# tigert1998/ray-tracing-cuda

Hardware: AMD Instinct MI355X
Metric: Mrays/s (higher is better)
Workload: dtype f32

## Files before the change

ray-tracing-cuda_amd/csrc/closest_hit.h:

```cpp
#pragma once

#ifdef RTMI_CHECK_MARGINS
__device__ inline bool aabb_hit_reference(const BvhNode &nd, V3 o, V3 d, double t_from, double t_to) {
  const float oo[3] = {o.x, o.y, o.z}, dd[3] = {d.x, d.y, d.z};
  for (int i = 0; i < 3; i++) {
    if (dd[i] == 0.f) continue;
    for (int s = 0; s < 2; s++) {
      const float tf = ((s == 0 ? nd.mn[i] : nd.mx[i]) - oo[i]) / dd[i];
      const double t = (double)tf;
      if (t != t || fabs(t) == (double)INFINITY) continue;
      if (!(t_from <= t && t <= t_to)) continue;
      const float pt[3] = {oo[0] + (float)t * dd[0], oo[1] + (float)t * dd[1], oo[2] + (float)t * dd[2]};
      bool inside = true;
      for (int a = 0; a < 3; a++)
        if (a != i && !(nd.mn[a] <= pt[a] && pt[a] <= nd.mx[a])) inside = false;
      if (inside) return true;
    }
  }
  return false;
}
template <typename T>
__device__ inline bool bvh_reference_walk(const SceneDev &sc, const BvhRec &br, V3 o, V3 d, T &t_to, int &face, float &fu,
                                          float &fv) {
  int stk_node[kRefDepthMax + 2], stk_first[kRefDepthMax + 2], stk_n[kRefDepthMax + 2];
  int sp = 1;
  stk_node[0] = br.root, stk_first[0] = 0, stk_n[0] = br.n_faces;
  bool hit = false;
  while (sp > 0) {
    sp--;
    const int node = stk_node[sp], first = stk_first[sp], n = stk_n[sp];
    const BvhNode nd = sc.nodes[node];
    if (node != br.root && !aabb_hit_reference(nd, o, d, 1e-3, (double)t_to)) continue;
    if (nd.right < 0) {
      for (int i = 0; i < n; i++) {
        const int fi = sc.face_of_orig[br.face_base + first + i];
        const FaceRec &f = sc.faces[fi];
        float t = 0.f, u = 0.f, v = 0.f;
        if (tri_test<T>(mk(f.p0[0], f.p0[1], f.p0[2]), mk(f.e1[0], f.e1[1], f.e1[2]), mk(f.e2[0], f.e2[1], f.e2[2]), o, d,
                        t_to, t, u, v))
          t_to = (T)t, face = fi, fu = u, fv = v, hit = true;
      }
    } else if (sp + 2 <= kRefDepthMax + 2) {
      const int mid = (n - 1) / 2;
      stk_node[sp] = nd.right, stk_first[sp] = first + mid + 1, stk_n[sp] = n - mid - 1;
      stk_node[sp + 1] = nd.left, stk_first[sp + 1] = first, stk_n[sp + 1] = mid + 1;
      sp += 2;
    }
  }
  return hit;
}
#endif

template <uint32_t M, bool PAIR = false>
__device__ __forceinline__ bool load_tri_pts(const SceneDev &sc, const float4 *s_tris, int rec, int which, V3 &p0, V3 &e1, V3 &e2) {
  float4 qa, qb, qc;
  bool present;
  if ((M & PIN_LDS_TABLES) || s_tris != nullptr) {
    const float4 *pp = s_tris + (size_t)rec * 3;
    if (trims_mul24(M)) {
      uint32_t at = (uint32_t)(uintptr_t)s_tris + __umul24((uint32_t)(PAIR ? rec - which : rec), 48u);
      asm volatile("" : "+v"(at));
      pp = (const float4 *)(const RT_LDS float4 *)(uintptr_t)at + (PAIR ? 3 * which : 0);
    }
    qa = load_lds<float4>(pp), qb = load_lds<float4>(pp + 1), qc = load_lds<float4>(pp + 2);
    present = !(__float_as_int(qc.y) & TRIPTS_ABSENT);
  } else {
    const float4 *pp = reinterpret_cast<const float4 *>(sc.tris + rec);
    qa = load_global<float4>(pp), qb = load_global<float4>(pp + 1), qc = load_global<float4>(pp + 2);
    const float4 qd = load_global<float4>(pp + 3);
    present = which == 0 || (__float_as_int(qd.y) & TRI_SECOND);
  }
  p0 = mk(qa.x, qa.y, qa.z), e1 = mk(qa.w, qb.x, qb.y), e2 = mk(qb.z, qb.w, qc.x);
  return present;
}

template <uint32_t F, bool OCC = false, uint32_t M = 0>
__device__ __forceinline__ Hit closest_hit(const SceneDev &sc, const BvhNode *s_nodes, int lds_nodes, const int *s_paths,
                                           int lds_paths, const float4 *s_tris, int *ll, uint16_t *cands, int *wl,
                                           unsigned long long *overflow, V3 o, V3 d, bool live, bool count_work
#ifdef RTMI_STATS
                                           , MeshStats &st
#endif
                                           , double t_start = INFINITY, double t_stop = INFINITY, bool *uncertain = nullptr
) {
  constexpr bool DT = (F & F_SPHERE) != 0;
  typedef typename TSel<DT>::type T;
  bool ok = false;
  T t_to = OCC ? (T)t_start : (T)INFINITY;
#define RTMI_DECIDED (OCC && ok && t_to <= (T)t_stop)
  uint32_t win = ID_NONE;
  int32_t aux = 0;
  int32_t work = 0;
  float bu = 0.f, bv = 0.f;

  double sa = 0.0, sa2 = 0.0;
  float saf = 0.f;
  if (F & F_SPHERE) {
    float la = len3(d);
    saf = la * la;
    sa = (double)saf;
    sa2 = 2 * sa;
  }

  const int lane = (int)(threadIdx.x & 63u);
  const bool det_safe = (M & PIN_DET_SAFE) || sc.det_safe != 0;
  constexpr bool SLAB = culls_by_slab(M);
  constexpr bool MINF = folds_by_min(M);
  constexpr bool VOTE = trims_votes(M);
  static_assert(!MINF || (!OCC && !DT && !(F & F_TEX)), "a key holds a binary32 t and the triangle's place, nothing else");
  const bool cull_list = (F & F_TRIS) && ((M & PIN_LDS_TABLES) || (ll != nullptr && sc.n_pairs >= kCullMinPairs));
  V3 cull_inv = splat(0.f), cull_klo = splat(0.f), cull_khi = splat(0.f);
  if ((F & F_TRIS) && cull_list) {
    const float ix = __builtin_amdgcn_rcpf(d.x), iy = __builtin_amdgcn_rcpf(d.y), iz = __builtin_amdgcn_rcpf(d.z);
    cull_inv = mk(fabsf(d.x) < 1e-30f ? copysignf(1e30f, d.x) : ix, fabsf(d.y) < 1e-30f ? copysignf(1e30f, d.y) : iy,
                  fabsf(d.z) < 1e-30f ? copysignf(1e30f, d.z) : iz);
    if (SLAB) {
      cull_klo = mk(-o.x * cull_inv.x, -o.y * cull_inv.y, -o.z * cull_inv.z);
    } else {
      const float delta = MESH_DIST_SLACK * (fmaxf(fmaxf(fabsf(o.x), fabsf(o.y)), fabsf(o.z)) + sc.list_mag);
      cull_klo = mk(-(o.x + delta) * cull_inv.x, -(o.y + delta) * cull_inv.y, -(o.z + delta) * cull_inv.z);
      cull_khi = mk(-(o.x - delta) * cull_inv.x, -(o.y - delta) * cull_inv.y, -(o.z - delta) * cull_inv.z);
    }
  }

  for (int ri = 0; ri < sc.n_runs; ri++) {
    if (OCC) {
      live = live && !RTMI_DECIDED;
      if (__builtin_amdgcn_ballot_w64(live) == 0ull) break;
    }
    const i32x4 rv = load_run(sc.runs, ri);
    Run run;
    run.kind = rv[0], run.first = rv[1], run.count = rv[2], run.pad = rv[3];
    if (live && run.kind == RUN_SKY) {
      const T ts = (T)1e9f;
      bool hit = ts <= t_to;
      bool acc = hit && (!ok || ts < t_to);
      ok = ok || acc;
      t_to = acc ? ts : t_to;
      win = acc ? make_id(RUN_SKY, 0) : win;
    }
    if ((F & F_TRIS) && run.kind == RUN_TRIS && cull_list) {
      const int pair0 = run.first >> 1;
      const float lo0 = T_FROM_F * kTimeLo;
      for (int c0 = 0; c0 < run.count; c0 += 32) {
        if (OCC && __builtin_amdgcn_ballot_w64(live && !RTMI_DECIDED) == 0ull) break;
        const int nc = run.count - c0 < 32 ? run.count - c0 : 32;
        const float hi0 = (float)t_to * kTimeHi + kTimeAbs;
        uint32_t mask = 0u;
        RTMI_STAT2(const unsigned long long tc0 = stat_now();)
#define RTMI_CULL_PAIR(bx)                                                                                                      \
  {                                                                                                                             \
    const float t0x = __builtin_fmaf(bx[0], cull_inv.x, cull_klo.x), t1x = __builtin_fmaf(bx[3], cull_inv.x, cull_khi.x); \
    const float t0y = __builtin_fmaf(bx[1], cull_inv.y, cull_klo.y), t1y = __builtin_fmaf(bx[4], cull_inv.y, cull_khi.y); \
    const float t0z = __builtin_fmaf(bx[2], cull_inv.z, cull_klo.z), t1z = __builtin_fmaf(bx[5], cull_inv.z, cull_khi.z); \
    const float en = fmaxf(fmaxf(fminf(t0x, t1x), fminf(t0y, t1y)), fminf(t0z, t1z));                                            \
    const float le = fminf(fminf(fmaxf(t0x, t1x), fmaxf(t0y, t1y)), fmaxf(t0z, t1z));                                            \
    cull_step(mask, fmaxf(lo0, en), fminf(hi0, le));                                                                            \
  }
#define RTMI_CULL_SLAB(bx)                                                                                                      \
  {                                                                                                                             \
    const float tcx = __builtin_fmaf(bx[0], cull_inv.x, cull_klo.x), tcy = __builtin_fmaf(bx[1], cull_inv.y, cull_klo.y),       \
                tcz = __builtin_fmaf(bx[2], cull_inv.z, cull_klo.z);                                                            \
    const float nx = __builtin_fmaf(-bx[3], fabsf(cull_inv.x), tcx), fx = __builtin_fmaf(bx[3], fabsf(cull_inv.x), tcx);        \
    const float ny = __builtin_fmaf(-bx[4], fabsf(cull_inv.y), tcy), fy = __builtin_fmaf(bx[4], fabsf(cull_inv.y), tcy);        \
    const float nz = __builtin_fmaf(-bx[5], fabsf(cull_inv.z), tcz), fz = __builtin_fmaf(bx[5], fabsf(cull_inv.z), tcz);        \
    const float en = fmaxf(fmaxf(nx, ny), nz), le = fminf(fminf(fx, fy), fz);                                                   \
    cull_step_nlt(mask, fminf(hi0, le), fmaxf(lo0, en));                                                                        \
  }
#define RTMI_CULL_ONE(bx)  \
  if (SLAB) RTMI_CULL_SLAB(bx) else RTMI_CULL_PAIR(bx)
        const PairBox *const recs = sc.pair_boxes;
        f32x8 A = load_pair_box(recs, pair0 + c0), B;
        int i = 0;
        for (; i + 1 < nc; i += 2) {
          __builtin_amdgcn_s_waitcnt(0xc07f);
          __builtin_amdgcn_sched_barrier(0);
          B = load_pair_box(recs, pair0 + c0 + i + 1);
          __builtin_amdgcn_sched_barrier(0);
          RTMI_CULL_ONE(A)
          __builtin_amdgcn_s_waitcnt(0xc07f);
          __builtin_amdgcn_sched_barrier(0);
          A = load_pair_box(recs, pair0 + c0 + i + 2);
          __builtin_amdgcn_sched_barrier(0);
          RTMI_CULL_ONE(B)
        }
        if (i < nc) {
          __builtin_amdgcn_s_waitcnt(0xc07f);
          __builtin_amdgcn_sched_barrier(0);
          RTMI_CULL_ONE(A)
        }
#undef RTMI_CULL_ONE
#undef RTMI_CULL_SLAB
#undef RTMI_CULL_PAIR
        mask = __brev(mask) >> (32 - nc);
        if (!live) mask = 0u;
        if (OCC && RTMI_DECIDED) mask = 0u;
        RTMI_STAT2(const unsigned long long tc1 = stat_now(); st.cyc[5] += tc1 - tc0;)
        RTMI_STAT(st.cull_bits += (unsigned)__popcll(__builtin_amdgcn_ballot_w64(true)) * 0u; { unsigned pc = __builtin_popcount(mask); for (int off = 32; off > 0; off >>= 1) pc += __shfl_down(pc, off); st.cull_bits += __builtin_amdgcn_readfirstlane(pc); } st.cull_rays += (unsigned)__popcll(__builtin_amdgcn_ballot_w64(true));)
#ifndef RTMI_OWN_FIRST
#define RTMI_OWN_FIRST 1
#endif
#if RTMI_OWN_FIRST
        if (wave_ballot_nz<VOTE>(mask) != 0ull) {
          if (mask != 0u) {
            const int bit = __builtin_ctz(mask);
            mask &= mask - 1u;
            const int rec = 2 * (pair0 + c0 + bit);
            V3 p0, e1, e2, p1, e1b, e2b;
            (void)load_tri_pts<M, true>(sc, s_tris, rec, 0, p0, e1, e2);
            const bool second = load_tri_pts<M, true>(sc, s_tris, rec + 1, 1, p1, e1b, e2b);
            float ta = 0.f, ua = 0.f, va = 0.f, tb = 0.f, ub = 0.f, vb = 0.f;
            const bool hit_a = tri_test_flat<T, VOTE>(p0, e1, e2, cross3(d, e2), o, d, t_to, ta, ua, va, det_safe);
            bool hit_b = false;
            if (second) hit_b = tri_test_flat<T, VOTE>(p1, e1b, e2b, cross3(d, e2b), o, d, t_to, tb, ub, vb, det_safe) && !hit_a;
            const float t = hit_a ? ta : tb;
            const bool acc = (hit_a || hit_b) && (!ok || (T)t < t_to);
            ok = ok || acc;
            t_to = acc ? (T)t : t_to;
            win = acc ? make_id(RUN_TRIS, run.first + 2 * (c0 + bit) + (hit_a ? 0 : 1)) : win;
            if (F & F_TEX) {
              bu = acc ? (hit_a ? ua : ub) : bu;
              bv = acc ? (hit_a ? va : vb) : bv;
            }
          }
        }
        if (OCC && RTMI_DECIDED) mask = 0u;
#endif
        {
          constexpr int RW = (F & F_TEX) ? 6 : 2;
          int *tasks = ll + 64 * 8, *results = ll + 64 * 8 + kListTasks(F);
          const int cnt = __builtin_popcount(mask);
          const int base = wave_prefix_excl(cnt);
          if (cnt != 0) {
            int *rr = ll + lane * 8;
            int w3 = 0, w7 = 0;
            if (DT) {
              const double td = (double)t_to;
              w3 = __double2loint(td), w7 = __double2hiint(td);
            } else {
              w3 = __float_as_int((float)t_to);
            }
            *reinterpret_cast<int4 *>(rr) = make_int4(__float_as_int(o.x), __float_as_int(o.y), __float_as_int(o.z), w3);
            *reinterpret_cast<int4 *>(rr + 4) = make_int4(__float_as_int(d.x), __float_as_int(d.y), __float_as_int(d.z), w7);
          }
          bool todo = cnt != 0;
          uint32_t left = (uint32_t)cnt;
#define RTMI_TODO_LANES (VOTE ? wave_ballot_nz<true>(left) : __builtin_amdgcn_ballot_w64(todo))
          while (RTMI_TODO_LANES != 0ull) {
            RTMI_STAT(st.cull_iters++;)
            const int lo_t = __builtin_amdgcn_readlane(base, __builtin_ctzll(RTMI_TODO_LANES));
            const bool now = (VOTE ? left != 0u : todo) && base + cnt - lo_t <= kListTasks(F);
            const unsigned long long now_lanes = VOTE ? RTMI_TODO_LANES & __builtin_amdgcn_sicmp(base + cnt - lo_t, kListTasks(F), 41)
                                                      : __builtin_amdgcn_ballot_w64(now);
            const int n_now = __builtin_amdgcn_readlane(base + cnt, 63 - __builtin_clzll(now_lanes)) - lo_t;
            RTMI_STAT(st.nnow_hist[(n_now - 1) >> 5 < 5 ? (n_now - 1) >> 5 : 5]++;)
            RTMI_STAT({
              int pc = now ? cnt : 0;
              for (int off = 32; off > 0; off >>= 1) pc = max(pc, __shfl_xor(pc, off));
              st.trip_hist[pc < 8 ? pc - 1 : 7]++;
            })
            int ln = lane;
            if (MINF) asm volatile("" : "+v"(ln));
            if (now) {
              int k = base - lo_t;
              for (uint32_t m = mask; m != 0u; m &= m - 1u) tasks[k++] = (lane << 5) | __builtin_ctz(m);
              if (MINF) results[2 * ln + 1] = -1;
            }
            wave_lds_fence();
            if (MINF) {
              bool flagged = false;
              for (int t0 = 0; t0 < 2 * n_now; t0 += 64) {
                const int ti = t0 + ln;
                if (ti < 2 * n_now) {
                  const int w = tasks[ti >> 1], which = ti & 1;
                  const int *orr = ll + (w >> 5) * 8;
                  const float4 r0 = *reinterpret_cast<const float4 *>(orr), r1 = *reinterpret_cast<const float4 *>(orr + 4);
                  const V3 ro = mk(r0.x, r0.y, r0.z), rd = mk(r1.x, r1.y, r1.z);
                  V3 p0, e1, e2;
                  const bool present = load_tri_pts<M>(sc, s_tris, 2 * (pair0 + c0 + (w & 31)) + which, which, p0, e1, e2);
                  float tt = 0.f, uu, vv;
                  bool hit = false;
                  if (present) hit = tri_test_flat<T, VOTE>(p0, e1, e2, cross3(rd, e2), ro, rd, (T)r0.w, tt, uu, vv, det_safe);
                  const int mine = hit ? __float_as_int(tt) : -1;
                  const int other = __builtin_amdgcn_update_dpp(mine, mine, 0xb1, 0xf, 0xf, false);
                  const bool yield = other != -1 && (which != 0 || __int_as_float(other) < tt);
                  flagged = flagged || (hit && yield && which == 0);
                  if (hit && !yield) {
                    const unsigned long long key = ((unsigned long long)(uint32_t)mine << 32) | (uint32_t)(2 * (w & 31) + which);
                    (void)__hip_atomic_fetch_min(reinterpret_cast<unsigned long long *>(results + 2 * (w >> 5)), key,
                                                 __ATOMIC_RELAXED, __HIP_MEMORY_SCOPE_WAVEFRONT);
                  }
                }
              }
              wave_lds_fence();
              const unsigned long long fl = __builtin_amdgcn_ballot_w64(flagged);
              if (fl == 0ull) {
                if (now) {
                  const int2 key = *reinterpret_cast<const int2 *>(results + 2 * ln);
                  const float t = __int_as_float(key.y);
                  const bool acc = key.y != -1 && (!ok || (T)t < t_to);
                  ok = ok || acc;
                  t_to = acc ? (T)t : t_to;
                  win = acc ? make_id(RUN_TRIS, run.first + 2 * c0 + key.x) : win;
                  todo = false, left = 0u;
                }
                wave_lds_fence();
                continue;
              }
              if (lane == 0) atomicAdd(overflow + (kOrderedTasksWord - 2), (unsigned long long)__popcll(fl));
            }
            for (int t0 = 0; t0 < 2 * n_now; t0 += 64) {
              const int ti = t0 + lane;
              if (ti < 2 * n_now) {
                const int w = tasks[ti >> 1], which = ti & 1;
                const int *orr = ll + (w >> 5) * 8;
                const float4 r0 = *reinterpret_cast<const float4 *>(orr), r1 = *reinterpret_cast<const float4 *>(orr + 4);
                T t0_to;
                if (DT) {
                  t0_to = (T)__hiloint2double(__float_as_int(r1.w), __float_as_int(r0.w));
                } else {
                  t0_to = (T)r0.w;
                }
                const V3 ro = mk(r0.x, r0.y, r0.z), rd = mk(r1.x, r1.y, r1.z);
                V3 p0, e1, e2;
                const bool present = load_tri_pts<M>(sc, s_tris, 2 * (pair0 + c0 + (w & 31)) + which, which, p0, e1, e2);
                float tt = 0.f, uu = 0.f, vv = 0.f;
                bool hit = false;
                if (present) hit = tri_test_flat<T, VOTE>(p0, e1, e2, cross3(rd, e2), ro, rd, t0_to, tt, uu, vv, det_safe);
                int *res = results + (ti >> 1) * RW;
                res[which] = hit ? __float_as_int(tt) : (int)0xffffffff;
                if (F & F_TEX) res[2 + 2 * which] = __float_as_int(uu), res[3 + 2 * which] = __float_as_int(vv);
              }
            }
            wave_lds_fence();
            RTMI_STAT2(const unsigned long long tc2 = stat_now();)
            if (now) {
              int k = base - lo_t;
              for (uint32_t m = mask; m != 0u; m &= m - 1u, k++) {
                const int tri = run.first + 2 * (c0 + __builtin_ctz(m));
                const int *res = results + k * RW;
                const int ia = res[0], ib = res[1];
                const float ta = __int_as_float(ia), tb = __int_as_float(ib);
                const bool hit_a = ia != (int)0xffffffff && (T)ta <= t_to;
                const bool hit_b = !hit_a && ib != (int)0xffffffff && (T)tb <= t_to;
                const float t = hit_a ? ta : tb;
                const bool acc = (hit_a || hit_b) && (!ok || (T)t < t_to);
                ok = ok || acc;
                t_to = acc ? (T)t : t_to;
                win = acc ? make_id(RUN_TRIS, tri + (hit_a ? 0 : 1)) : win;
                if (F & F_TEX) {
                  bu = acc ? __int_as_float(hit_a ? res[2] : res[4]) : bu;
                  bv = acc ? __int_as_float(hit_a ? res[3] : res[5]) : bv;
                }
              }
              todo = false, left = 0u;
            }
            wave_lds_fence();
            RTMI_STAT2(st.cyc[7] += stat_now() - tc2;)
          }
#undef RTMI_TODO_LANES
        }
        RTMI_STAT2(st.cyc[6] += stat_now() - tc1;)
      }
    } else if ((F & F_TRIS) && live && run.kind == RUN_TRIS) {
      const HotTri *base = sc.tris + run.first;
      f32x16 A = load_hot_tri(base, 0);
      for (int i = 0; i < run.count; i++) {
        if (OCC && __builtin_amdgcn_ballot_w64(!RTMI_DECIDED) == 0ull) break;
        __builtin_amdgcn_s_waitcnt(0xc07f);
        __builtin_amdgcn_sched_barrier(0);
        const f32x16 B = load_hot_tri(base, 2 * i + 1);
        __builtin_amdgcn_sched_barrier(0);
        float t = 0.f, u = 0.f, v = 0.f;
        const V3 pv_a = cross3(d, mk(A[6], A[7], A[8]));
        const bool hit_a = tri_test_flat<T>(mk(A[0], A[1], A[2]), mk(A[3], A[4], A[5]), mk(A[6], A[7], A[8]), pv_a, o, d,
                                            t_to, t, u, v, det_safe);
        {
          bool acc = hit_a && (!ok || (T)t < t_to);
          ok = ok || acc;
          t_to = acc ? (T)t : t_to;
          win = acc ? make_id(RUN_TRIS, run.first + 2 * i) : win;
          if (F & F_TEX) {
            bu = acc ? u : bu;
            bv = acc ? v : bv;
          }
        }
        __builtin_amdgcn_s_waitcnt(0xc07f);
        __builtin_amdgcn_sched_barrier(0);
        A = load_hot_tri(base, 2 * i + 2);
        __builtin_amdgcn_sched_barrier(0);
        if (__float_as_int(B[13]) & TRI_SECOND) {
          V3 pv_b = pv_a;
          if (!(__float_as_int(B[13]) & TRI_SAME_E2)) pv_b = cross3(d, mk(B[6], B[7], B[8]));
          bool hit_b = tri_test_flat<T>(mk(B[0], B[1], B[2]), mk(B[3], B[4], B[5]), mk(B[6], B[7], B[8]), pv_b, o, d,
                                        t_to, t, u, v, det_safe);
          hit_b = hit_b && !hit_a;
          bool acc = hit_b && (!ok || (T)t < t_to);
          ok = ok || acc;
          t_to = acc ? (T)t : t_to;
          win = acc ? make_id(RUN_TRIS, run.first + 2 * i + 1) : win;
          if (F & F_TEX) {
            bu = acc ? u : bu;
            bv = acc ? v : bv;
          }
        }
      }
    }
    bool grouped_done = false;
    if ((F & F_SGROUP) && run.kind == RUN_SPHERE && run.pad >= 0 && cands != nullptr) {
      const int n_groups = (run.count + kSphGroupSize - 1) / kSphGroupSize;
      uint16_t *my_cands = cands + lane * kSphCand;
      int *tasks = ll + 64 * 8, *results = ll + 64 * 8 + kListTasks(F);
      int ccnt = 0;
      bool have = false;
      double best_v = 0.0;
      int best_idx = 0;
      {
        int *rr = ll + lane * 8;
        *reinterpret_cast<int4 *>(rr) = make_int4(__float_as_int(o.x), __float_as_int(o.y), __float_as_int(o.z), __float_as_int(saf));
        *reinterpret_cast<int4 *>(rr + 4) = make_int4(__float_as_int(d.x), __float_as_int(d.y), __float_as_int(d.z), 0);
      }
      const float sdelta = kSphDistSlack * fmaxf(fmaxf(fabsf(o.x), fabsf(o.y)), fabsf(o.z));
      const float six = __builtin_amdgcn_rcpf(d.x), siy = __builtin_amdgcn_rcpf(d.y), siz = __builtin_amdgcn_rcpf(d.z);
      const V3 s_inv = mk(fabsf(d.x) < 1e-30f ? copysignf(1e30f, d.x) : six, fabsf(d.y) < 1e-30f ? copysignf(1e30f, d.y) : siy,
                          fabsf(d.z) < 1e-30f ? copysignf(1e30f, d.z) : siz);
      const V3 s_klo = mk(-(o.x + sdelta) * s_inv.x, -(o.y + sdelta) * s_inv.y, -(o.z + sdelta) * s_inv.z);
      const V3 s_khi = mk(-(o.x - sdelta) * s_inv.x, -(o.y - sdelta) * s_inv.y, -(o.z - sdelta) * s_inv.z);
      const float s_lo0 = T_FROM_F * kTimeLo, s_hi0 = (float)t_to * kTimeHi + kTimeAbs;
      const int member0 = __float_as_int(load_sph_group(sc.sph_groups, run.pad)[6]);
      auto flush = [&]() {
        const int cnt = ccnt;
        const int base = wave_prefix_excl(cnt);
        bool todo = cnt != 0;
        while (__builtin_amdgcn_ballot_w64(todo) != 0ull) {
          const int lo_t = __builtin_amdgcn_readlane(base, __builtin_ctzll(__builtin_amdgcn_ballot_w64(todo)));
          const bool now = todo && base + cnt - lo_t <= kListTasks(F);
          const int n_now = __builtin_amdgcn_readlane(base + cnt, 63 - __builtin_clzll(__builtin_amdgcn_ballot_w64(now))) - lo_t;
          if (now)
            for (int j = 0; j < cnt; j++) tasks[base - lo_t + j] = (lane << 16) | (int)my_cands[j];
          wave_lds_fence();
          for (int t0 = 0; t0 < n_now; t0 += 64) {
            const int ti = t0 + lane;
            if (ti < n_now) {
              const int w = tasks[ti];
              const int *orr = ll + (w >> 16) * 8;
              const float4 r0 = *reinterpret_cast<const float4 *>(orr), r1 = *reinterpret_cast<const float4 *>(orr + 4);
              const SphMember *mp = sc.sph_members + member0 + (w & 0xffff);
              const float4 m0 = *reinterpret_cast<const float4 *>(mp);
              const int4 m1 = *reinterpret_cast<const int4 *>(reinterpret_cast<const char *>(mp) + 16);
              const double r2 = __hiloint2double(m1.w, m1.z);
              const V3 ro = mk(r0.x, r0.y, r0.z), rd = mk(r1.x, r1.y, r1.z);
              const double tsa = (double)r0.w, tsa2 = 2 * tsa;
              const V3 oc = ro - mk(m0.x, m0.y, m0.z);
              const double b = (double)(2.0f * dot3(rd, oc));
              const float lc = len3(oc);
              const double c = (double)(lc * lc) - r2;
              const double disc = b * b - 4 * tsa * c;
              double v = __hiloint2double(0x7ff80000, 0);
              if (!(disc < 0)) {
                const double sq = sqrt(disc);
                const double t1 = (-b - sq) / tsa2;
                if (1e-3 <= t1) {
                  v = t1;
                } else {
                  const double t2 = (-b + sq) / tsa2;
                  if (1e-3 <= t2) v = t2;
                }
              }
              int *res = results + ti * 3;
              res[0] = __double2loint(v), res[1] = __double2hiint(v), res[2] = m1.x;
            }
          }
          wave_lds_fence();
          if (now) {
            for (int j = 0; j < cnt; j++) {
              const int *res = results + (base - lo_t + j) * 3;
              const double v = __hiloint2double(res[1], res[0]);
              const int idx = res[2];
              if (v == v && (!have || v < best_v || (v == best_v && idx < best_idx))) have = true, best_v = v, best_idx = idx;
            }
            todo = false;
          }
          wave_lds_fence();
        }
        ccnt = 0;
      };
      int *counts = reinterpret_cast<int *>(cands + 64 * kSphCand);
      counts[lane] = 0;
      bool over = false;
      for (int g0 = 0; g0 < n_groups; g0 += 32) {
        const int ngc = n_groups - g0 < 32 ? n_groups - g0 : 32;
        uint32_t gmask = 0u;
        f32x8 G = load_sph_group(sc.sph_groups, run.pad + g0);
        for (int g = 0; g < ngc; g++) {
          __builtin_amdgcn_s_waitcnt(0xc07f);
          __builtin_amdgcn_sched_barrier(0);
          const f32x8 gb = G;
          G = load_sph_group(sc.sph_groups, run.pad + g0 + g + 1);
          __builtin_amdgcn_sched_barrier(0);
          const float t0x = __builtin_fmaf(gb[0], s_inv.x, s_klo.x), t1x = __builtin_fmaf(gb[3], s_inv.x, s_khi.x);
          const float t0y = __builtin_fmaf(gb[1], s_inv.y, s_klo.y), t1y = __builtin_fmaf(gb[4], s_inv.y, s_khi.y);
          const float t0z = __builtin_fmaf(gb[2], s_inv.z, s_klo.z), t1z = __builtin_fmaf(gb[5], s_inv.z, s_khi.z);
          const float en = fmaxf(fmaxf(fminf(t0x, t1x), fminf(t0y, t1y)), fminf(t0z, t1z));
          const float le = fminf(fminf(fmaxf(t0x, t1x), fmaxf(t0y, t1y)), fmaxf(t0z, t1z));
          cull_step(gmask, fmaxf(s_lo0, en), fminf(s_hi0, le));
        }
        gmask = live ? __brev(gmask) >> (32 - ngc) : 0u;
        const int cnt = __builtin_popcount(gmask);
        const int base = wave_prefix_excl(cnt);
        bool todo = cnt != 0;
        while (__builtin_amdgcn_ballot_w64(todo) != 0ull) {
          const int lo_t = __builtin_amdgcn_readlane(base, __builtin_ctzll(__builtin_amdgcn_ballot_w64(todo)));
          const bool now = todo && base + cnt - lo_t <= kListTasks(F);
          const int n_now = __builtin_amdgcn_readlane(base + cnt, 63 - __builtin_clzll(__builtin_amdgcn_ballot_w64(now))) - lo_t;
          if (now) {
            int k = base - lo_t;
            for (uint32_t m = gmask; m != 0u; m &= m - 1u) tasks[k++] = (lane << 16) | (g0 + __builtin_ctz(m));
          }
          wave_lds_fence();
          for (int t0 = 0; t0 < n_now; t0 += 64) {
            const int ti = t0 + lane;
            if (ti < n_now) {
              const int w = tasks[ti];
              const int owner = w >> 16;
              const int *orr = ll + owner * 8;
              const float4 r0 = *reinterpret_cast<const float4 *>(orr), r1 = *reinterpret_cast<const float4 *>(orr + 4);
              const V3 ro = mk(r0.x, r0.y, r0.z), rd = mk(r1.x, r1.y, r1.z);
              const float ta4 = 4.0f * r0.w;
              const int2 gr = *reinterpret_cast<const int2 *>(reinterpret_cast<const char *>(sc.sph_groups + run.pad + (w & 0xffff)) + 24);
              const int rel = gr.x - member0;
              const float4 *mp = reinterpret_cast<const float4 *>(sc.sph_members + gr.x);
#pragma unroll 4
              for (int i = 0; i < kSphGroupSize; i++) {
                if (i < gr.y) {
                  const float4 mb = mp[2 * i];
                  const V3 oc = ro - mk(mb.x, mb.y, mb.z);
                  const float bf = 2.0f * dot3(rd, oc);
                  const float oc2 = dot3(oc, oc);
                  const float bb = bf * bf;
                  const float disc_f = bb - ta4 * (oc2 - mb.w);
                  const float mag = bb + ta4 * (oc2 + mb.w);
                  if (!(disc_f < -kSphDiscRel * mag)) {
                    const int slot = atomicAdd(&counts[owner], 1);
                    if (slot < kSphCand) {
                      cands[owner * kSphCand + slot] = (uint16_t)(rel + i);
                    } else {
                      over = true;
                    }
                  }
                }
              }
            }
          }
          wave_lds_fence();
          if (now) todo = false;
        }
      }
      const bool overflowed = __any(over);
      if (!overflowed) {
        ccnt = counts[lane];
        flush();
        if (have) {
          const bool hit = best_v <= (double)t_to;
          const bool acc = hit && (!ok || best_v < (double)t_to);
          ok = ok || acc;
          t_to = acc ? (T)best_v : t_to;
          win = acc ? make_id(RUN_SPHERE, best_idx) : win;
        }
        grouped_done = true;
      }
    }
    if ((F & F_SPHERE) && live && run.kind == RUN_SPHERE && !grouped_done) {
      f32x8 nxt = load_sphere(sc.spheres, run.first);
      for (int i = 0; i < run.count; i++) {
        if (OCC && __builtin_amdgcn_ballot_w64(!RTMI_DECIDED) == 0ull) break;
        __builtin_amdgcn_s_waitcnt(0xc07f);
        __builtin_amdgcn_sched_barrier(0);
        const f32x8 cur = nxt;
        nxt = load_sphere(sc.spheres, run.first + i + 1);
        __builtin_amdgcn_sched_barrier(0);
        const double r2 = __hiloint2double(__float_as_int(cur[7]), __float_as_int(cur[6]));
        V3 oc = o - mk(cur[0], cur[1], cur[2]);
        const float bf = 2.0f * dot3(d, oc);
        {
          const float oc2 = dot3(oc, oc), r2f = (float)r2;
          const float disc_f = bf * bf - 4.0f * saf * (oc2 - r2f);
          const float mag = bf * bf + 4.0f * saf * (oc2 + r2f);
          if (!__any(!(disc_f < -kSphDiscRel * mag) && !RTMI_DECIDED)) continue;
        }
        double b = (double)bf;
        float lc = len3(oc);
        double c = (double)(lc * lc) - r2;
        double disc = b * b - 4 * sa * c;
        bool hit = false;
        double t = 0.0;
        if (!(disc < 0)) {
          double sq = sqrt(disc);
          t = (-b - sq) / sa2;
          hit = (1e-3 <= t && t <= (double)t_to);
          if (!hit) {
            t = (-b + sq) / sa2;
            hit = (1e-3 <= t && t <= (double)t_to);
          }
        }
        bool acc = hit && (!ok || t < (double)t_to);
        ok = ok || acc;
        t_to = acc ? (T)t : t_to;
        win = acc ? make_id(RUN_SPHERE, run.first + i) : win;
      }
    }
#if defined(RTMI_ABLATE) && RTMI_ABLATE == 3
    if (false) {
#else
    if ((F & F_BVH) && run.kind == RUN_BVH) {
#endif
      const V3 inv_d = mk(safe_inverse(d.x), safe_inverse(d.y), safe_inverse(d.z));
      int *rr = wl + lane * kMeshRayWords;
      for (int i = 0; i < run.count; i++) {
        if (OCC && __builtin_amdgcn_ballot_w64(live && !RTMI_DECIDED) == 0ull) break;
        BvhRec br;
        {
          const i32x16 bw = load_bvh_rec(sc.bvhs, run.first + i);
          br.root = bw[0], br.mat = bw[1], br.has_uv = bw[2], br.face_base = bw[3], br.sub_root = bw[4];
          br.mag = __int_as_float(bw[5]);
          br.ref_depth = bw[6], br.path_base = bw[7];
#pragma unroll
          for (int c = 0; c < 3; c++) br.root_mn[c] = __int_as_float(bw[8 + c]), br.root_mx[c] = __int_as_float(bw[11 + c]);
          br.n_faces = bw[14], br.slack_exp = bw[15];
        }
        T bt_to = t_to;
        bool bhit = false;
        int bface = 0;
        float fu = 0.f, fv = 0.f;
#ifdef RTMI_CHECK_MARGINS
        if (wl == nullptr) {
          if (live) bhit = bvh_reference_walk<T>(sc, br, o, d, bt_to, bface, fu, fv);
          const bool acc = bhit && (!ok || bt_to < t_to);
          ok = ok || acc;
          t_to = acc ? bt_to : t_to;
          win = acc ? make_id(RUN_BVH, bface) : win;
          aux = acc ? run.first + i : aux;
          bu = acc ? fu : bu;
          bv = acc ? fv : bv;
          continue;
        }
#endif
        bool have_prev = false;
        uint32_t prev_code = 0u, entered = 0u;
        uint32_t lo_code = 0u;
        bool need = live && !RTMI_DECIDED;
        bool listed = false;
#ifndef RTMI_MESH_PRETEST
#define RTMI_MESH_PRETEST 1
#endif
#if RTMI_MESH_PRETEST
        if (br.ref_depth > 0) {
          BvhNode rn;
          rn.mn[0] = br.root_mn[0], rn.mn[1] = br.root_mn[1], rn.mn[2] = br.root_mn[2];
          rn.mx[0] = br.root_mx[0], rn.mx[1] = br.root_mx[1], rn.mx[2] = br.root_mx[2];
          const float diag = fmaxf(fmaxf(rn.mx[0] - rn.mn[0], rn.mx[1] - rn.mn[1]), rn.mx[2] - rn.mn[2]);
          const float pad = 1e-3f * diag + 1e-4f * br.mag +
                            ldexpf(0x1p-15f * (fmaxf(fmaxf(fabsf(o.x), fabsf(o.y)), fabsf(o.z)) + br.mag), br.slack_exp);
          need = need && slab_touch(rn, pad, o, inv_d, T_FROM_F * kTimeLo, (float)bt_to * kTimeHi + kTimeAbs);
        }
#endif
        while (__ballot(need) != 0ull) {
          RTMI_STAT(const unsigned long long ts0 = stat_now();)
          mesh_search<T, DT>(sc, br.sub_root, sc.tops + (size_t)(run.first + i) * kTopEntries, br.mag, wl, need, o, d, inv_d,
                             bt_to, lo_code, overflow, count_work
#ifdef RTMI_STATS
                             , st
#endif
          );
          if (!DT && count_work && need) work += rr[7];
          RTMI_STAT(const unsigned long long ts1 = stat_now(); st.cyc[2] += ts1 - ts0;)
          RTMI_STAT(const unsigned long long tr0 = stat_now(); (void)tr0;)
          uint32_t cut = kCodeNone;
          int cnt = 0;
          int4 hs[kHitSlots];
#pragma unroll
          for (int j = 0; j < kHitSlots; j++) hs[j] = make_int4((int)kCodeNone, 0, 0, 0);
          if (need) {
            const int4 head = *reinterpret_cast<const int4 *>(rr + 12);
            cnt = head.x, cut = (uint32_t)head.y;
            const int4 wa = *reinterpret_cast<const int4 *>(rr + 16), wb = *reinterpret_cast<const int4 *>(rr + 20),
                       wc = *reinterpret_cast<const int4 *>(rr + 24);
            const int4 e4[kHitSlots] = {make_int4(wa.x, wa.y, wa.z, 0), make_int4(wa.w, wb.x, wb.y, 0),
                                        make_int4(wb.z, wb.w, wc.x, 0), make_int4(wc.y, wc.z, wc.w, 0)};
#pragma unroll
            for (int j = 0; j < kHitSlots; j++)
              if (j < cnt && (uint32_t)e4[j].x < cut) hs[j] = e4[j];
          }
#define RTMI_ORDER(A, B)                                        \
  {                                                             \
    const bool sw = (uint32_t)hs[B].x < (uint32_t)hs[A].x;      \
    const int4 lo_ = sw ? hs[B] : hs[A], hi_ = sw ? hs[A] : hs[B]; \
    hs[A] = lo_, hs[B] = hi_;                                   \
  }
          RTMI_ORDER(0, 1) RTMI_ORDER(2, 3) RTMI_ORDER(0, 2) RTMI_ORDER(1, 3) RTMI_ORDER(1, 2)
#undef RTMI_ORDER
          int nleaf = 0;
#pragma unroll
          for (int j = 0; j < kHitSlots; j++) nleaf += (uint32_t)hs[j].x != kCodeNone ? 1 : 0;
          if (OCC) listed = listed || nleaf > 0;
          const int depth_r = br.ref_depth;
          const int log_d = depth_r < 8 ? 3 : depth_r < 16 ? 4 : 5;
          const int rows_max = (kMeshStackWords - 64) >> log_d < 64 ? (kMeshStackWords - 64) >> log_d : 64;
          const int base = wave_prefix_excl(nleaf);
          int *leaves = wl + 64 * kMeshRayWords;
          int *times = leaves + 64;
#if defined(RTMI_ABLATE) && RTMI_ABLATE == 4
          bool todo = false;
#else
          bool todo = nleaf > 0 && depth_r > 0;
#endif
          RTMI_STAT3(unsigned long long tr1 = stat_now(); st.cyc[5] += tr1 - ts1;)
          while (__builtin_amdgcn_ballot_w64(todo) != 0ull) {
            const int lo = __builtin_amdgcn_readlane(base, __builtin_ctzll(__builtin_amdgcn_ballot_w64(todo)));
            const bool now = todo && base + nleaf - lo <= rows_max;
            const int n_rows = __builtin_amdgcn_readlane(base + nleaf, 63 - __builtin_clzll(__builtin_amdgcn_ballot_w64(now))) - lo;
            if (now) {
#pragma unroll
              for (int k = 0; k < kHitSlots; k++)
                if (k < nleaf) leaves[base - lo + k] = (lane << 26) | hs[k].x;
            }
            wave_lds_fence();
            RTMI_STAT3(const unsigned long long tr2 = stat_now(); st.cyc[6] += tr2 - tr1;)
            const int n_now = n_rows << log_d;
            for (int t0 = 0; t0 < n_now; t0 += 64) {
              const int t = t0 + lane, lvl = t & ((1 << log_d) - 1);
              if (t < n_now && lvl <= depth_r) {
                const int w = leaves[t >> log_d];
                const int pi = br.path_base + (w & (kMeshMaxNodes - 1)) * (depth_r + 1) + lvl;
                const int ni = pi < lds_paths ? s_paths[pi] : sc.leaf_paths[pi];
                float m = __int_as_float(lvl == 0 ? ni : (int)0xffffffff);
                if (lvl != 0 && ni >= 0) {
                  const int *orr = wl + (int)((unsigned)w >> 26) * kMeshRayWords;
                  const float4 r0 = *reinterpret_cast<const float4 *>(orr + 0), r1 = *reinterpret_cast<const float4 *>(orr + 4);
                  BvhNode nd;
                  if (ni < lds_nodes) {
                    nd = s_nodes[ni];
                  } else {
                    nd = sc.nodes[ni];
                  }
#if defined(RTMI_ABLATE) && RTMI_ABLATE == 5
                  m = nd.mn[0] * r0.x + r1.x;
#else
                  m = aabb_crossing_time(nd, mk(r0.x, r0.y, r0.z), mk(r1.x, r1.y, r1.z));
#endif
                }
                times[t] = __float_as_int(m);
              }
            }
            wave_lds_fence();
            RTMI_STAT3(const unsigned long long tr3 = stat_now(); st.cyc[7] += tr3 - tr2;)
            if (__builtin_amdgcn_ballot_w64(now) != 0ull) {
#pragma unroll
              for (int k = 0; k < kHitSlots; k++) {
                if (__builtin_amdgcn_ballot_w64(now && k < nleaf) == 0ull) break;
                const bool mine = now && k < nleaf;
                const int *row = times + (mine ? (base - lo + k) << log_d : 0);
                uint32_t code = 0u, valid = 0u, below = 0u;
                for (int c = 0; c <= depth_r; c += 8) {
                  const int4 ma = *reinterpret_cast<const int4 *>(row + c), mb = *reinterpret_cast<const int4 *>(row + c + 4);
                  const int mv[8] = {ma.x, ma.y, ma.z, ma.w, mb.x, mb.y, mb.z, mb.w};
                  if (c == 0) code = (uint32_t)ma.x;
#pragma unroll
                  for (int j = 0; j < 8; j++) {
                    const uint32_t bit = 0x80000000u >> ((c + j - 1) & 31);
                    const bool in_row = c + j >= 1 && c + j <= depth_r;
                    valid |= in_row && mv[j] != (int)0xffffffff ? bit : 0u;
#if defined(RTMI_ABLATE) && RTMI_ABLATE == 1
                    below |= in_row ? bit : 0u;
#else
                    below |= in_row && (T)__int_as_float(mv[j]) <= bt_to ? bit : 0u;
#endif
                  }
                }
                const int shared = have_prev ? __clz((int)(prev_code ^ code)) : 0;
                const uint32_t common = shared ? 0xffffffffu << (32 - shared) : 0u;
                const uint32_t pass = (entered & common) | (below & ~common);
                const uint32_t fail = valid & ~pass;
                const int upto = fail ? __clz((int)fail) : __popc(valid);
                const uint32_t walked = upto ? 0xffffffffu << (32 - upto) : 0u;
                const uint32_t bits = (entered & common) | (walked & ~common);
                if (mine) {
                  have_prev = true;
                  prev_code = code;
                  entered = bits;
                  const T tj = (T)__int_as_float(hs[k].z);
                  if (fail == 0u && tj <= bt_to) {
                    bt_to = tj;
                    bhit = true;
                    bface = hs[k].y;
                  }
                }
              }
              if (now) todo = false;
            }
            wave_lds_fence();
            RTMI_STAT3(tr1 = stat_now(); st.cyc[8] += tr1 - tr3;)
          }
#if defined(RTMI_ABLATE) && RTMI_ABLATE == 4
          if (nleaf > 0) {
#else
          if (nleaf > 0 && depth_r == 0) {
#endif
#pragma unroll
            for (int k = 0; k < kHitSlots; k++) {
              if (k < nleaf) {
                const T tj = (T)__int_as_float(hs[k].z);
                if (tj <= bt_to) bt_to = tj, bhit = true, bface = hs[k].y;
              }
            }
          }
          need = need && cut != kCodeNone;
          if (OCC) need = need && !(bhit && bt_to <= (T)t_stop);
          lo_code = cut;
          RTMI_STAT(st.cyc[3] += stat_now() - ts1;)
        }
        if (OCC && uncertain != nullptr && listed && !bhit && t_start != (double)INFINITY) *uncertain = true;
        if (!OCC && bhit && (F & F_TEX)) {
          const FaceRec f = sc.faces[bface];
          float t = 0.f;
          const V3 fe2 = mk(f.e2[0], f.e2[1], f.e2[2]);
          (void)tri_test_flat<T>(mk(f.p0[0], f.p0[1], f.p0[2]), mk(f.e1[0], f.e1[1], f.e1[2]), fe2, cross3(d, fe2), o, d,
                                 bt_to, t, fu, fv);
        }
        bool acc = bhit && (!ok || bt_to < t_to);
        ok = ok || acc;
        t_to = acc ? bt_to : t_to;
        win = acc ? make_id(RUN_BVH, bface) : win;
        aux = acc ? run.first + i : aux;
        bu = acc ? fu : bu;
        bv = acc ? fv : bv;
      }
    }
  }
#undef RTMI_DECIDED
  Hit h;
  h.ok = ok;
  h.t = (float)t_to;
  h.win = win;
  h.aux = aux;
  h.u = bu;
  h.v = bv;
  h.work = work;
  return h;
}
```

ray-tracing-cuda_amd/csrc/kernels.h:

```cpp
#pragma once
#include <hip/hip_runtime.h>
#include <stdint.h>

#include <vector>

#include "../../include/rtmi.h"
#include "scene_dev.h"

#define RTMI_KERNEL_MAX_DEPTH 64

namespace rtmi {

#include "path_list.h"

int64_t frame_pixel_of(const FrameDev &fr, int rank, int64_t q);

hipError_t launch_rng_init(uint64_t seed, const FrameDev &fr, const uint32_t *d_jump, uint32_t *d_states,
                           hipStream_t stream, int64_t first = -1);

uint32_t pick_variant(uint32_t features);
int render_occupancy(uint32_t variant, const SceneDev &sc, const FrameDev &fr, int threads, bool fast_path = false);
struct RenderTuning {
  int schedule;
  int blocks_per_cu;
  int threads;
  int sparse_stride;
  int exclusive;
  int outlier_x10;
  int head_pct[3];
  int probe_spp;
  int promote;
  int first_pass;
  int cost_probe;
  int lane_stride;
  int plan;
  int prio_every;
  int fast_path;
  int head_classes;
  int first_prio;
  int fetch_batch, fetch_batch_first;
};

enum : uint32_t {
  PIN_NIBBLE_IDS = 1u << 0,
  PIN_LDS_TABLES = 1u << 1,
  PIN_UNSIGNED = 1u << 2,
  PIN_DET_SAFE = 1u << 3,
  PIN_POW2_FRAME = 1u << 4,
  PIN_EVERY_LANE = 1u << 5,
  PIN_PRIORITIES = 1u << 6,
  PIN_CHAINS = 1u << 7,
  PIN_QUEUE = 1u << 8,
  PIN_DIFFUSE = 1u << 9,
};
constexpr uint32_t kFastCommon = PIN_NIBBLE_IDS | PIN_LDS_TABLES | PIN_UNSIGNED | PIN_DET_SAFE | PIN_POW2_FRAME |
                                 PIN_EVERY_LANE | PIN_PRIORITIES;
constexpr uint32_t kFastChains = kFastCommon | PIN_CHAINS;
constexpr uint32_t kFastQueue = kFastCommon | PIN_QUEUE;
constexpr bool defers_unit(uint32_t m) { return (m & kFastCommon) == kFastCommon; }
constexpr bool culls_by_slab(uint32_t m) { return (m & kFastCommon) == kFastCommon; }
constexpr bool folds_by_min(uint32_t m) { return (m & kFastCommon) == kFastCommon; }
#ifndef RTMI_TRIM
#define RTMI_TRIM 7
#endif
constexpr bool trims_votes(uint32_t m) { return (RTMI_TRIM & 1) && (m & kFastCommon) == kFastCommon; }
constexpr bool trims_mul24(uint32_t m) { return (RTMI_TRIM & 2) && (m & kFastCommon) == kFastCommon; }
constexpr bool trims_fold_rgb(uint32_t m) { return (RTMI_TRIM & 4) && (m & kFastCommon) == kFastCommon; }
#ifndef RTMI_DIFFUSE
#define RTMI_DIFFUSE 5
#endif
constexpr bool diffuse_scatter(uint32_t m) { return (RTMI_DIFFUSE & 1) && (m & PIN_DIFFUSE) && (m & kFastCommon) == kFastCommon; }
constexpr bool diffuse_restarts(uint32_t m) { return (RTMI_DIFFUSE & 4) && diffuse_scatter(m); }
inline uint32_t render_pins(uint32_t fast, const SceneDev &sc) { return fast != 0u && sc.diffuse_only ? fast | PIN_DIFFUSE : fast; }
constexpr int kFoldRgbOff = 512;
constexpr int kFoldRgbBytes = 256;
constexpr int kOrderedTasksWord = 16;
struct FastPathFacts {
  int enabled;
  uint32_t variant;
  int n_mats;
  int mats_in_lds;
  int pairs_in_lds;
  int unsigned_colours;
  int det_safe;
  int width, height;
  int lane_stride;
  int priorities;
  int chains;
  int resumed;
  int tile_cost;
};
uint32_t fast_path_mode(const FastPathFacts &f);
FastPathFacts fast_path_facts(uint32_t variant, const SceneDev &sc, const FrameDev &fr, int threads, int enabled);
bool slab_reach_covers(float list_mag, const CameraDev &cam);
size_t render_lds_bytes(uint32_t variant, const SceneDev &sc, const FrameDev &fr, int threads);
struct SchedPlan {
  const uint32_t *tile_order = nullptr;
  uint32_t *visit_counts = nullptr;
  const uint32_t *sparse_items = nullptr;
  const uint32_t *head_list = nullptr;
  const uint32_t *probe_marks = nullptr;
  int probe_spp = 2;
  uint32_t *prio_tab = nullptr;
  const uint32_t *tile_cost = nullptr;
  const int32_t *chain_next = nullptr;
  const uint32_t *chain_fut = nullptr;
  const int32_t *chain_first = nullptr;
  uint32_t *claims = nullptr;
  int plan_simds = 0, plan_rounds = 0;
};
size_t render_params_bytes();
hipError_t launch_render(uint32_t variant, const SceneDev &sc, const FrameDev &fr, uint32_t *d_states, float *d_out,
                         uint32_t *d_ray_counts, unsigned long long *d_counters, const SchedPlan &plan, bool probe,
                         uint32_t fast, int blocks, int threads, const RenderTuning &tune, void *d_params, hipStream_t stream);
constexpr int kHeadCap = 16384;
hipError_t launch_tile_order(uint32_t *d_ray_counts, int n_tiles, uint32_t *d_cost, uint32_t *d_meta,
                             uint32_t *d_order, uint32_t *d_head, uint32_t sparse_cap, int grid_waves, int outlier_x10,
                             const int head_pct[3], hipStream_t stream);

hipError_t launch_quarter_order(const uint32_t *d_order, const uint32_t *d_work, const uint32_t *d_rays, int n_tiles,
                                uint32_t *d_qcost, uint32_t *d_qsorted, uint32_t *d_qmax, uint32_t *d_qmap, hipStream_t stream);

hipError_t launch_chain_plan(const uint32_t *d_order, const uint32_t *d_cost, int n_tiles, int simds, int rounds, int spp,
                             int probe_spp, int32_t *d_first, int32_t *d_next, uint32_t *d_fut, hipStream_t stream);

hipError_t launch_untile(const FrameDev &fr, const float *d_tiles, float *d_image, hipStream_t stream);
hipError_t launch_untile_u32(const FrameDev &fr, const uint32_t *d_tiles, uint32_t *d_image, hipStream_t stream);
hipError_t launch_post(float *d_img, int64_t n, int spp, hipStream_t stream);
uint32_t pick_query_variant(uint32_t features);
hipError_t launch_query(uint32_t variant, const SceneDev &sc, const QueryDev &qd, int n_cu, int64_t n, const float *d_o,
                        const float *d_d, const float *d_t_max, int32_t *d_hits, unsigned long long *d_abandoned,
                        unsigned long long *d_check, hipStream_t stream);
hipError_t launch_occlusion(uint32_t variant, const SceneDev &sc, const float near_lo[3], const float near_hi[3],
                            float near_short, int n_cu, int64_t n, const PathList *list, const float *d_o, const float *d_d,
                            const float *d_t_max, uint8_t *d_occluded, unsigned long long *d_counts,
                            unsigned long long *d_check, hipStream_t stream);
constexpr size_t kCallParamsOffset = 256;
hipError_t launch_trace(uint32_t variant, const SceneDev &sc, bool tex_layers, int n_cu, int64_t n, int max_depth,
                        const float *d_o, const float *d_d, uint32_t *d_states, float *d_radiance,
                        uint32_t *d_ray_counts, unsigned long long *d_work, hipStream_t stream);
hipError_t launch_bounce(uint32_t variant, const SceneDev &sc, const QueryDev &qd, int n_cu, int64_t n, const PathList *list,
                         float *d_o, float *d_d, uint32_t *d_states, float *d_emitted, float *d_attenuation, int32_t *d_hits,
                         uint32_t *d_steps, unsigned long long *d_work, hipStream_t stream);
size_t path_compact_scratch_bytes(int64_t n_list);
hipError_t launch_path_compact(int64_t n, const float *d_origins, const float *d_dirs, const PathList &in, uint32_t *d_list_out,
                               uint32_t *d_count_out, uint32_t *d_scratch, hipStream_t stream);
static inline int64_t cdiv(int64_t a, int64_t b) { return (a + b - 1) / b; }
inline unsigned list_grid(uint32_t n_list, int threads, int n_cu, int blocks_per_cu) {
  const int64_t want = ((int64_t)n_list + threads - 1) / threads, cap = (int64_t)(n_cu > 0 ? n_cu : 1) * blocks_per_cu;
  return (unsigned)(want < cap ? want : cap);
}
hipError_t launch_path_fold(int64_t n, int layers, const float *d_dirs, const uint32_t *d_steps, const float *d_emitted,
                            const float *d_attenuation, float *d_radiance, hipStream_t stream);
struct Scene;
struct LightRec;
struct DirectArgs;
void build_light_table(const Scene &s, std::vector<rtmi_light> *lights, std::vector<uint32_t> *light_mats);
void light_records(const std::vector<rtmi_light> &lights, std::vector<LightRec> *recs, std::vector<float> *cdf);
hipError_t launch_direct_sample(const DirectArgs &a, int n_cu, hipStream_t stream);
struct DirectMisArgs;
void build_hit_light_map(const std::vector<rtmi_light> &lights, std::vector<int32_t> *map, int32_t *n_entries);
hipError_t launch_direct_sample_mis(const DirectMisArgs &a, int n_cu, hipStream_t stream);
hipError_t launch_direct_sample_sph(const DirectMisArgs &a, bool mis, int n_cu, hipStream_t stream);
hipError_t launch_path_fold_direct(int64_t n, int layers, const float *d_dirs, const uint32_t *d_steps, const float *d_emitted,
                                   const float *d_attenuation, const float *d_direct, const uint8_t *d_occluded,
                                   float *d_radiance, hipStream_t stream);
hipError_t launch_budget(uint32_t variant, const SceneDev &sc, bool tex_layers, int n_cu, const FrameDev &fr,
                         const uint32_t *d_budget, uint32_t *d_states, float *d_sum, float *d_sq, uint32_t *d_samples,
                         uint32_t *d_ray_counts, const FeatureBufs *feat, unsigned long long *d_work, hipStream_t stream);
hipError_t launch_resolve_features(const FrameDev &fr, const FeatureBufs &sums, const uint32_t *d_samples,
                                   const FeatureBufs &out, hipStream_t stream);
hipError_t launch_budget_plan(const FrameDev &fr, int min_samples, int max_samples, int step, float tolerance, float floor,
                              const float *d_sum, const float *d_sq, const uint32_t *d_samples, uint32_t *d_budget,
                              unsigned long long *d_totals, hipStream_t stream);
hipError_t launch_resolve(const FrameDev &fr, const float *d_sum, const uint32_t *d_samples, int post, float *d_tiles,
                          hipStream_t stream);
hipError_t launch_resolve_variance(const FrameDev &fr, const float *d_sum, const float *d_sq, const uint32_t *d_samples,
                                   float *d_var, hipStream_t stream);
struct DenoiseCall {
  int height, width, iterations, normal_squarings, demodulate;
  float sigma_color, sigma_depth;
  const float *color, *variance, *albedo, *normal, *depth, *alpha;
  float *out, *out_variance;
  void *scratch;
};
size_t denoise_scratch_bytes(int height, int width);
hipError_t launch_denoise(const DenoiseCall &d, hipStream_t stream);
struct AccumulateCall {
  int height, width;
  float normal_min, depth_tolerance, min_blend;
  float e[3], h[3], v[3], p[3];
  float prev_p[3], r[3][3];
  const float *color, *variance, *normal, *depth, *alpha;
  const void *history_in;
  void *history_out;
  float *out, *out_variance, *out_length;
};
size_t history_bytes(int height, int width);
hipError_t launch_accumulate(const AccumulateCall &c, hipStream_t stream);
hipError_t launch_camera_rays(const FrameDev &fr, const CameraDev &cam, const float w[3], int kind, float fov,
                              const uint32_t *d_budget, uint32_t sample, uint32_t *d_states, float *d_origins,
                              float *d_dirs, hipStream_t stream);
hipError_t launch_sample_add(const FrameDev &fr, const uint32_t *d_budget, uint32_t sample, const float *d_radiance,
                             const uint32_t *d_trace_counts, float *d_sum, float *d_sq, uint32_t *d_samples,
                             uint32_t *d_ray_counts, hipStream_t stream);
struct AdvanceCall {
  const uint32_t *budget;
  PathList list;
  float *origins, *dirs;
  uint32_t *states, *steps;
  const float *emitted, *attenuation;
  float *emitted_stack, *attenuation_stack;
  uint32_t *cursor;
  float *sum, *sq;
  uint32_t *samples, *ray_counts;
  unsigned long long *counts;
};
hipError_t launch_path_advance(const FrameDev &fr, const CameraDev &cam, const float w[3], int kind, float fov,
                               const AdvanceCall &c, int n_cu, hipStream_t stream);
#ifdef RTMI_STATS
hipError_t copy_wave_stats(unsigned long long *host, size_t bytes);
#endif
#ifdef RTMI_CHECK_MARGINS
hipError_t launch_add_one(unsigned long long *d_word, hipStream_t stream);
#endif
hipError_t launch_arithmetic_selftest(unsigned long long *d_bad, hipStream_t stream);

}
```

Baseline: 39190.

## Test both triangles of a pair per lane in full deferred task rounds

In the deferred min-fold task list, rounds with many pending pairs now assign one whole triangle pair per lane instead of one triangle per lane. Each lane tests both triangles against its ray and posts an atomic-min key. The remaining tail still runs one triangle per lane. A narrow LDS load variant reads only the needed words of the third float4, and a pair-round planning helper is added. The aim is fewer rounds and less per-task overhead, at the cost of longer serial work per lane and possible divergence.

```diff
diff --git a/ray-tracing-cuda_amd/csrc/closest_hit.h b/ray-tracing-cuda_amd/csrc/closest_hit.h
--- a/ray-tracing-cuda_amd/csrc/closest_hit.h
+++ b/ray-tracing-cuda_amd/csrc/closest_hit.h
@@ -51,7 +51,7 @@
 }
 #endif
 
-template <uint32_t M, bool PAIR = false>
+template <uint32_t M, bool PAIR = false, bool NARROW = false>
 __device__ __forceinline__ bool load_tri_pts(const SceneDev &sc, const float4 *s_tris, int rec, int which, V3 &p0, V3 &e1, V3 &e2) {
   float4 qa, qb, qc;
   bool present;
@@ -62,7 +62,13 @@
       asm volatile("" : "+v"(at));
       pp = (const float4 *)(const RT_LDS float4 *)(uintptr_t)at + (PAIR ? 3 * which : 0);
     }
-    qa = load_lds<float4>(pp), qb = load_lds<float4>(pp + 1), qc = load_lds<float4>(pp + 2);
+    qa = load_lds<float4>(pp), qb = load_lds<float4>(pp + 1);
+    if (NARROW) {
+      const float2 q2 = which == 0 ? make_float2(*(const RT_LDS float *)(pp + 2), 0.f) : load_lds<float2>(pp + 2);
+      qc = make_float4(q2.x, q2.y, 0.f, 0.f);
+    } else {
+      qc = load_lds<float4>(pp + 2);
+    }
     present = !(__float_as_int(qc.y) & TRIPTS_ABSENT);
   } else {
     const float4 *pp = reinterpret_cast<const float4 *>(sc.tris + rec);
@@ -73,6 +79,32 @@
   p0 = mk(qa.x, qa.y, qa.z), e1 = mk(qa.w, qb.x, qb.y), e2 = mk(qb.z, qb.w, qc.x);
   return present;
 }
+
+#define RTMI_PAIR_TEST(rec_, o_, d_, t_to_, SHARED)                                                                             \
+  V3 p0, e1, e2, p1, e1b, e2b;                                                                                                  \
+  (void)load_tri_pts<M, true, SHARED>(sc, s_tris, (rec_), 0, p0, e1, e2);                                                       \
+  bool second = false;                                                                                                          \
+  if (!(SHARED)) second = load_tri_pts<M, true, SHARED>(sc, s_tris, (rec_) + 1, 1, p1, e1b, e2b);                               \
+  float ta = 0.f, ua = 0.f, va = 0.f, tb = 0.f, ub = 0.f, vb = 0.f;                                                             \
+  const bool hit_a = tri_test_flat<T, VOTE>(p0, e1, e2, cross3(d_, e2), o_, d_, t_to_, ta, ua, va, det_safe);                   \
+  bool hit_b = false;                                                                                                           \
+  if (SHARED) {                                                                                                                 \
+    asm volatile("" : "+v"(ta));                                                                                                \
+    second = load_tri_pts<M, true, SHARED>(sc, s_tris, (rec_) + 1, 1, p1, e1b, e2b);                                            \
+    hit_b = tri_test_flat<T, VOTE>(p1, e1b, e2b, cross3(d_, e2b), o_, d_, t_to_, tb, ub, vb, det_safe) && second;               \
+  } else if (second) {                                                                                                          \
+    hit_b = tri_test_flat<T, VOTE>(p1, e1b, e2b, cross3(d_, e2b), o_, d_, t_to_, tb, ub, vb, det_safe) && !hit_a;               \
+  }
+
+#if defined(RTMI_CHECK_MARGINS) && !defined(RTMI_STATS)
+#define RTMI_COUNT_ROUND(word) \
+  if (PAIRS && ln == 0) atomicAdd(overflow + ((word) - 2), 1ull);
+#define RTMI_COUNT_PAIR_FLAG(cond) \
+  if (cond) atomicAdd(overflow + (kPairFlagsWord - 2), 1ull);
+#else
+#define RTMI_COUNT_ROUND(word)
+#define RTMI_COUNT_PAIR_FLAG(cond)
+#endif
 
 template <uint32_t F, bool OCC = false, uint32_t M = 0>
 __device__ __forceinline__ Hit closest_hit(const SceneDev &sc, const BvhNode *s_nodes, int lds_nodes, const int *s_paths,
@@ -107,6 +139,8 @@
   constexpr bool SLAB = culls_by_slab(M);
   constexpr bool MINF = folds_by_min(M);
   constexpr bool VOTE = trims_votes(M);
+  constexpr bool PAIRS = pairs_full_rounds(M) && kPairRoundMin < kListTasks(F);
+  static_assert(!PAIRS || MINF, "a pair round posts keys");
   static_assert(!MINF || (!OCC && !DT && !(F & F_TEX)), "a key holds a binary32 t and the triangle's place, nothing else");
   const bool cull_list = (F & F_TRIS) && ((M & PIN_LDS_TABLES) || (ll != nullptr && sc.n_pairs >= kCullMinPairs));
   V3 cull_inv = splat(0.f), cull_klo = splat(0.f), cull_khi = splat(0.f);
@@ -206,13 +240,7 @@
             const int bit = __builtin_ctz(mask);
             mask &= mask - 1u;
             const int rec = 2 * (pair0 + c0 + bit);
-            V3 p0, e1, e2, p1, e1b, e2b;
-            (void)load_tri_pts<M, true>(sc, s_tris, rec, 0, p0, e1, e2);
-            const bool second = load_tri_pts<M, true>(sc, s_tris, rec + 1, 1, p1, e1b, e2b);
-            float ta = 0.f, ua = 0.f, va = 0.f, tb = 0.f, ub = 0.f, vb = 0.f;
-            const bool hit_a = tri_test_flat<T, VOTE>(p0, e1, e2, cross3(d, e2), o, d, t_to, ta, ua, va, det_safe);
-            bool hit_b = false;
-            if (second) hit_b = tri_test_flat<T, VOTE>(p1, e1b, e2b, cross3(d, e2b), o, d, t_to, tb, ub, vb, det_safe) && !hit_a;
+            RTMI_PAIR_TEST(rec, o, d, t_to, false)
             const float t = hit_a ? ta : tb;
             const bool acc = (hit_a || hit_b) && (!ok || (T)t < t_to);
             ok = ok || acc;
@@ -269,7 +297,34 @@
             wave_lds_fence();
             if (MINF) {
               bool flagged = false;
-              for (int t0 = 0; t0 < 2 * n_now; t0 += 64) {
+              int done = 0;
+              if (PAIRS) {
+                for (; pair_round_due(n_now, done, kPairRoundMin); done += 64) {
+                  RTMI_COUNT_ROUND(kPairRoundsWord)
+                  const int ti = done + ln;
+                  if (ti < n_now) {
+                    const int w0 = tasks[ti];
+                    const int *orr = ll + (w0 >> 5) * 8;
+                    const float4 r0 = *reinterpret_cast<const float4 *>(orr), r1 = *reinterpret_cast<const float4 *>(orr + 4);
+                    const V3 ro = mk(r0.x, r0.y, r0.z), rd = mk(r1.x, r1.y, r1.z);
+                    RTMI_PAIR_TEST(2 * (pair0 + c0 + (w0 & 31)), ro, rd, (T)r0.w, true)
+                    const bool second_nearer = hit_a && hit_b && tb < ta;
+                    flagged = flagged || second_nearer;
+                    RTMI_COUNT_PAIR_FLAG(second_nearer)
+                    if ((hit_a || hit_b) && !second_nearer) {
+                      int tj = ti;
+                      asm volatile("" : "+v"(tj));
+                      const int w = tasks[tj];
+                      const unsigned long long key = ((unsigned long long)(uint32_t)__float_as_int(hit_a ? ta : tb) << 32) |
+                                                     (uint32_t)(2 * (w & 31) + (hit_a ? 0 : 1));
+                      (void)__hip_atomic_fetch_min(reinterpret_cast<unsigned long long *>(results + 2 * (w >> 5)), key,
+                                                   __ATOMIC_RELAXED, __HIP_MEMORY_SCOPE_WAVEFRONT);
+                    }
+                  }
+                }
+              }
+              for (int t0 = 2 * done; t0 < 2 * n_now; t0 += 64) {
+                RTMI_COUNT_ROUND(kTriRoundsWord)
                 const int ti = t0 + ln;
                 if (ti < 2 * n_now) {
                   const int w = tasks[ti >> 1], which = ti & 1;
@@ -359,6 +414,9 @@
             RTMI_STAT2(st.cyc[7] += stat_now() - tc2;)
           }
 #undef RTMI_TODO_LANES
+#undef RTMI_PAIR_TEST
+#undef RTMI_COUNT_ROUND
+#undef RTMI_COUNT_PAIR_FLAG
         }
         RTMI_STAT2(st.cyc[6] += stat_now() - tc1;)
       }
diff --git a/ray-tracing-cuda_amd/csrc/kernels.h b/ray-tracing-cuda_amd/csrc/kernels.h
--- a/ray-tracing-cuda_amd/csrc/kernels.h
+++ b/ray-tracing-cuda_amd/csrc/kernels.h
@@ -60,6 +60,12 @@
 constexpr bool defers_unit(uint32_t m) { return (m & kFastCommon) == kFastCommon; }
 constexpr bool culls_by_slab(uint32_t m) { return (m & kFastCommon) == kFastCommon; }
 constexpr bool folds_by_min(uint32_t m) { return (m & kFastCommon) == kFastCommon; }
+#ifndef RTMI_PAIR_ROUND_MIN
+#define RTMI_PAIR_ROUND_MIN 32
+#endif
+constexpr int kPairRoundMin = RTMI_PAIR_ROUND_MIN;
+constexpr bool pairs_full_rounds(uint32_t m) { return (m & kFastCommon) == kFastCommon; }
+#include "pair_rounds.h"
 #ifndef RTMI_TRIM
 #define RTMI_TRIM 7
 #endif
@@ -75,6 +81,7 @@
 constexpr int kFoldRgbOff = 512;
 constexpr int kFoldRgbBytes = 256;
 constexpr int kOrderedTasksWord = 16;
+constexpr int kPairRoundsWord = 37, kTriRoundsWord = 38, kPairFlagsWord = 39;
 struct FastPathFacts {
   int enabled;
   uint32_t variant;
diff --git a/ray-tracing-cuda_amd/csrc/pair_rounds.h b/ray-tracing-cuda_amd/csrc/pair_rounds.h
--- /dev/null
+++ b/ray-tracing-cuda_amd/csrc/pair_rounds.h
@@ -0,0 +1,12 @@
+#pragma once
+
+constexpr bool pair_round_due(int n_now, int done, int pair_min) { return n_now - done > pair_min; }
+
+inline int pair_round_plan(int n_now, int pair_min, int cap, int *first, int *count, int *pair) {
+  int r = 0, done = 0;
+  for (; pair_round_due(n_now, done, pair_min); done += 64, r++)
+    if (r < cap) first[r] = done, count[r] = n_now - done < 64 ? n_now - done : 64, pair[r] = 1;
+  for (int t0 = 2 * done; t0 < 2 * n_now; t0 += 64, r++)
+    if (r < cap) first[r] = t0 / 2, count[r] = 2 * n_now - t0 < 64 ? (2 * n_now - t0) / 2 : 32, pair[r] = 0;
+  return r;
+}
```

Measured after the change: 40730, median of 6. +3.9%, better.
